# kehlert/ellp

Measured on AMD Instinct MI355X. Metric: simplex pivots/sec (dense LP, primal, tableau resident in HBM), higher is better.
Workload: dtype f64

## Files before the change

### ellp_amd/_engine.py

```python
import ctypes as C
import os

import numpy as np

_HERE = os.path.dirname(os.path.abspath(__file__))
LIB_PATH = os.environ.get("ELLP_HIP_LIB") or os.path.join(_HERE, "libellp_hip.so")

OPTIMAL, INFEASIBLE, UNBOUNDED, MAXITER = 0, 1, 2, 3
ERR_BAD_DIMS, ERR_SINGULAR, ERR_NAN, ERR_DEVICE, ERR_ARG, ERR_PANIC = -1, -2, -3, -4, -5, -6
STATUS_NAME = {0: "optimal", 1: "infeasible", 2: "unbounded", 3: "maxiter", -1: "err_bad_dims",
               -2: "err_singular", -3: "err_nan", -4: "err_device", -5: "err_arg", -6: "err_panic"}
MAX_ITER_NONE = 2**64 - 1
ENGINE_PRIMAL, ENGINE_DUAL = 0, 1
FLAG_DENSE_PRICING, FLAG_DUAL_MAX_VIOLATION, FLAG_PRIMAL_STEEPEST_EDGE, FLAG_NO_CERTIFY, FLAG_DUAL_BOUND_FLIPPING = 1, 2, 4, 8, 16
K_NAMES = ["price", "select", "ftran", "ratio", "update", "btran", "refactor", "dleave", "dprice",
           "dselect", "dupdate", "event_cost"]
K_COUNT = 12
TAP_U, TAP_R, TAP_D, TAP_BINV, TAP_KEY, TAP_ALPHA, TAP_STATE = range(7)
TAP_SE_GAMMA = 7


class Opts(C.Structure):
    _fields_ = [("max_iter", C.c_uint64), ("eps", C.c_double), ("device", C.c_int32),
                ("refactor_period", C.c_int32), ("btran_mode", C.c_int32),
                ("poll_interval", C.c_int32), ("profile", C.c_int32), ("use_graph", C.c_int32),
                ("pipeline", C.c_int32), ("trace_len", C.c_int32), ("partial_segments", C.c_int32),
                ("flags", C.c_int32)]


class Stats(C.Structure):
    _fields_ = [("iters", C.c_uint64), ("pivots", C.c_uint64), ("bound_flips", C.c_uint64),
                ("refactors", C.c_uint64), ("obj", C.c_double), ("t_loop_s", C.c_double),
                ("t_setup_s", C.c_double), ("kernel_ms", C.c_double * K_COUNT),
                ("kernel_calls", C.c_uint64 * K_COUNT)]

    def as_dict(self):
        d = {k: getattr(self, k) for k in ("iters", "pivots", "bound_flips", "refactors", "obj",
                                           "t_loop_s", "t_setup_s")}
        d["kernel_ms"] = {K_NAMES[i]: self.kernel_ms[i] for i in range(K_COUNT) if self.kernel_calls[i]}
        d["kernel_calls"] = {K_NAMES[i]: self.kernel_calls[i] for i in range(K_COUNT) if self.kernel_calls[i]}
        return d


EXCHANGE_FN = C.CFUNCTYPE(C.c_int, C.c_void_p, C.c_void_p, C.c_int64, C.c_int)


class EllpHipError(RuntimeError):
    def __init__(self, status, msg):
        super().__init__(f"{STATUS_NAME.get(status, status)}: {msg}")
        self.status = status
        self.msg = msg


_lib = None
_PROBLEM_ARGS = [C.c_int64, C.c_int64, C.c_int64, C.c_void_p, C.c_void_p, C.c_void_p, C.c_void_p,
                 C.c_void_p, C.c_void_p, C.c_void_p, C.c_void_p, C.c_int64, C.c_void_p, C.c_void_p,
                 C.c_int64]


def lib():
    global _lib
    if _lib is not None:
        return _lib
    if not os.path.exists(LIB_PATH):
        raise ImportError(
            f"{LIB_PATH} is missing: the HIP engine is the only compute path of ellp_amd. "
            "Build it with `python -m ellp_amd.build` (hipcc --offload-arch=gfx950).")
    L = C.CDLL(LIB_PATH, mode=C.RTLD_GLOBAL)
    L.ellp_default_opts.argtypes = [C.POINTER(Opts)]
    L.ellp_hip_device_count.restype = C.c_int
    L.ellp_hip_abi_version.restype = C.c_int
    tail = [C.POINTER(Opts), C.POINTER(Stats), C.c_char_p, C.c_size_t]
    L.ellp_primal_solve_with_initial.restype = C.c_int
    L.ellp_primal_solve_with_initial.argtypes = _PROBLEM_ARGS + tail
    L.ellp_dual_solve_with_initial.restype = C.c_int
    L.ellp_dual_solve_with_initial.argtypes = _PROBLEM_ARGS + [C.c_void_p, C.c_void_p] + tail
    L.ellp_batch_solve_with_initial.restype = C.c_int
    L.ellp_batch_solve_with_initial.argtypes = [C.c_int, C.c_int64, C.c_void_p, C.POINTER(Opts), C.c_void_p, C.c_void_p,
                                                C.c_char_p, C.c_size_t]
    L.ellp_batch_primal_solve.restype = C.c_int
    L.ellp_batch_primal_solve.argtypes = [C.c_int64, C.c_void_p, C.POINTER(Opts), C.c_void_p, C.c_char_p, C.c_size_t]
    L.ellp_batch_primal_info.restype = None
    L.ellp_batch_primal_info.argtypes = [C.c_void_p]
    L.ellp_batch_dual_phase1_start.restype = C.c_int
    L.ellp_batch_dual_phase1_start.argtypes = [C.c_int64, C.c_void_p, C.POINTER(Opts), C.c_void_p, C.c_void_p, C.c_char_p,
                                               C.c_size_t]
    L.ellp_engine_create.restype = C.c_int
    L.ellp_engine_create.argtypes = ([C.c_int] + _PROBLEM_ARGS + [C.c_void_p, C.c_void_p] +
                                     [C.POINTER(Opts), C.POINTER(C.c_void_p), C.c_char_p, C.c_size_t])
    L.ellp_engine_plan.restype = C.c_int
    L.ellp_engine_plan.argtypes = [C.c_int, C.c_int64, C.c_int64, C.POINTER(Opts), C.c_int, C.c_void_p, C.c_int64, C.c_char_p, C.c_size_t]
    L.ellp_engine_run.restype = C.c_int
    L.ellp_engine_run.argtypes = [C.c_void_p, C.c_uint64, C.POINTER(Stats), C.c_char_p, C.c_size_t]
    L.ellp_engine_read_point.restype = C.c_int
    L.ellp_engine_read_point.argtypes = [C.c_void_p] + [C.c_void_p] * 6 + [C.c_char_p, C.c_size_t]
    L.ellp_engine_tap.restype = C.c_int64
    L.ellp_engine_tap.argtypes = [C.c_void_p, C.c_int, C.c_void_p, C.c_int64]
    L.ellp_engine_refactor.restype = C.c_int
    L.ellp_engine_refactor.argtypes = [C.c_void_p, C.c_char_p, C.c_size_t]
    L.ellp_engine_refresh.restype = C.c_double
    L.ellp_engine_refresh.argtypes = [C.c_void_p]
    L.ellp_engine_inverse_residual.restype = C.c_double
# ... 558 lines not shown
```

### ellp_amd/csrc/engine/ellp_engine.hip

```cpp
#include <hip/hip_runtime.h>
#include <dlfcn.h>
#include <rccl/rccl.h>

#include <algorithm>
#include <chrono>
#include <cmath>
#include <cstdarg>
#include <cstdint>
#include <cstdio>
#include <cstdlib>
#include <cstring>
#include <limits>
#include <memory>
#include <mutex>
#include <optional>
#include <vector>

#include "ellp_hip.h"
#include "ellp_lu_dev.h"

namespace {

constexpr int ST_RUNNING = 100;
constexpr int ST_NEED_MAINT = 101;
// ... 1699 lines not shown
    } else {
        const double theta_d = st->s_theta_d, delta = st->s_delta;
        const double theta_p = delta / d_r;
        const double *rho = src + r * a.ld;
        if (blockIdx.x == 0) {
        for (int64_t j0 = tid; j0 < a.nN; j0 += 4 * 256) {
            int64_t v[4];
            double al[4], dv[4];
#pragma unroll
            for (int k = 0; k < 4; ++k) {
                const int64_t j = j0 + 256 * k;
                const bool ok = j < a.nN && j != q;
                v[k] = ok ? a.N_index[j] : -1;
                al[k] = ok ? a.xc.r(j) : 0.0;
            }
#pragma unroll
            for (int k = 0; k < 4; ++k) dv[k] = v[k] >= 0 ? a.dd[v[k]] : 0.0;
#pragma unroll
            for (int k = 0; k < 4; ++k)
                if (v[k] >= 0) a.dd[v[k]] = dv[k] - theta_d * al[k];
        }
        return;
        }
        if (blockIdx.x == 1) {
            const int64_t lv = st->s_lv;
            for (int64_t i = tid; i < m; i += 256) a.y[i] = a.y[i] + theta_d * rho[i];
            swap_columns(a.A_N, a.A_B, q, r, a.ld, tid);
            if (tid == 0) {
                a.dd[lv] = -theta_d;
                a.dd[jq] = 0.0;
                a.N_index[q] = lv;
                a.Nb[q] = (uint8_t)st->s_side;
                const double tc = a.c_N[q];
                a.c_N[q] = a.c_B[r];
                a.c_B[r] = tc;
            }
            return;
        }
        for (int64_t i = tid; i < m; i += 256) {
            const int64_t bi = a.B_index[i];
            a.x[bi] = a.x[bi] - theta_p * a.d[i];
        }
        __syncthreads();
        if (tid == 0) {
            a.x[jq] = a.x[jq] + theta_p;
            st->obj = st->obj + theta_d * delta;
            a.B_index[r] = jq;
            st->cur = cur ^ 1;
            st->pivots += 1;
            st->iters += 1;
            trace_put(a.trace, st->iters, st->obj);
            if (d_r != d_r || theta_p != theta_p) st->status = ELLP_ERR_NAN;
        }
        __syncthreads();
        find_leaving(a.B_index, a.x, a.kind, a.lb, a.ub, a.eps, m, tid, s_tmp, st, a.maxviol);
        if (tid == 0 && tiny_pivot && st->status == ST_RUNNING) st->tiny = 1;
    }
    STAMP(2, 4);
}

struct DLeaveArgs {
    const double *x, *lb, *ub;
    const uint8_t *kind;
    const int64_t *B_index;
    DevState *st;
    int64_t m;
    double eps;
    int maxviol;
};
__global__ __launch_bounds__(256) void k_dleave(DLeaveArgs a) {
    __shared__ long long s_tmp[4];
    if (a.st->status != ST_RUNNING) return;
    find_leaving(a.B_index, a.x, a.kind, a.lb, a.ub, a.eps, a.m, threadIdx.x, s_tmp, a.st, a.maxviol);
}

struct BtranArgs {
    const double *W0, *W1, *c_B;
    double *upart, *u, *u_alt;
    DevState *st;
    int64_t m, ld;
    int rows_per_tile, ntiles;
};

__device__ __forceinline__ void btran_part_body(BtranArgs a, unsigned bx, unsigned by) {
    if (a.st->status != ST_RUNNING) return;
    const int64_t half = a.ld >> 1;
    const int64_t j2 = (int64_t)bx * 256 + threadIdx.x;
    const int64_t i0 = (int64_t)by * a.rows_per_tile;
    const int64_t i1 = (i0 + a.rows_per_tile < a.m) ? i0 + a.rows_per_tile : a.m;
    double2 acc = make_double2(0.0, 0.0);
    if (j2 < half) {
        const double2 *W2 = reinterpret_cast<const double2 *>(a.st->cur ? a.W1 : a.W0);
        for (int64_t i = i0; i < i1; ++i) {
            const double ci = a.c_B[i];
            if (ci != 0.0) {
                const double2 w = W2[i * half + j2];
                acc.x = fma(ci, w.x, acc.x);
                acc.y = fma(ci, w.y, acc.y);
            }
        }
        reinterpret_cast<double2 *>(a.upart)[(int64_t)by * half + j2] = acc;
    }
}
__global__ __launch_bounds__(256) void k_btran_part(BtranArgs a) { btran_part_body(a, blockIdx.x, blockIdx.y); }
__device__ __forceinline__ void btran_reduce_body(BtranArgs a, unsigned bx) {
    if (a.st->status != ST_RUNNING) return;
    const int64_t j = (int64_t)bx * 256 + threadIdx.x;
    if (j >= a.ld) return;
    double s = 0.0;
    int t = 0;
    for (; t + 8 <= a.ntiles; t += 8) {
        double v[8];
#pragma unroll
        for (int k = 0; k < 8; ++k) v[k] = a.upart[(int64_t)(t + k) * a.ld + j];
#pragma unroll
        for (int k = 0; k < 8; ++k) s += v[k];
    }
    for (; t < a.ntiles; ++t) s += a.upart[(int64_t)t * a.ld + j];
    (a.st->usel ? a.u_alt : a.u)[j] = s;
}
__global__ __launch_bounds__(256) void k_btran_reduce(BtranArgs a) { btran_reduce_body(a, blockIdx.x); }


__device__ __forceinline__ double nanmax(double a, double b) { return (a != a) ? a : ((b > a || b != b) ? b : a); }

struct DriftArgs {
    const double *A_B, *A_N, *d;
    const double *aq_cur;
    double *upart;
    DevState *st;
    int64_t m, ld;
    int cols_per_tile, ntiles;
    double tol;
};
__global__ __launch_bounds__(256) void k_drift_part(DriftArgs a) {
    if (a.st->status != ST_RUNNING || a.st->pp_skip) return;
    const int64_t half = a.ld >> 1;
    const int64_t i2 = (int64_t)blockIdx.x * 256 + threadIdx.x;
    const int64_t k0 = (int64_t)blockIdx.y * a.cols_per_tile;
    const int64_t k1 = (k0 + a.cols_per_tile < a.m) ? k0 + a.cols_per_tile : a.m;
    if (i2 >= half) return;
    const double2 *AB2 = reinterpret_cast<const double2 *>(a.A_B);
    double2 acc = make_double2(0.0, 0.0);
    for (int64_t k = k0; k < k1; ++k) {
        const double dk = a.d[k];
        const double2 c = AB2[k * half + i2];
        acc.x = fma(dk, c.x, acc.x);
        acc.y = fma(dk, c.y, acc.y);
    }
    reinterpret_cast<double2 *>(a.upart)[(int64_t)blockIdx.y * half + i2] = acc;
}
__global__ __launch_bounds__(1024) void k_drift_reduce(DriftArgs a) {
    __shared__ double s_r[16], s_s[16];
    DevState *st = a.st;
    if (st->status != ST_RUNNING || st->pp_skip) return;
    const int tid = threadIdx.x, lane = tid & 63, wave = tid >> 6;
    const double sgn = st->s_at_lower ? -1.0 : 1.0;
    const double *aq = a.aq_cur ? a.aq_cur : a.A_N + st->s_q * a.ld;
    double res = 0.0, scale = 0.0;
    for (int64_t i = tid; i < a.m; i += 1024) {
        double t = 0.0;
        for (int k = 0; k < a.ntiles; ++k) t += a.upart[(int64_t)k * a.ld + i];
        const double q = aq[i];
        res = nanmax(res, fabs(sgn * t - q));
        scale = nanmax(scale, fabs(q));
    }
#pragma unroll
    for (int o = 32; o > 0; o >>= 1) {
        res = nanmax(res, __shfl_xor(res, o));
        scale = nanmax(scale, __shfl_xor(scale, o));
    }
    if (lane == 0) {
        s_r[wave] = res;
        s_s[wave] = scale;
    }
    __syncthreads();
    if (tid == 0) {
        for (int w = 1; w < 16; ++w) {
            res = nanmax(res, s_r[w]);
            scale = nanmax(scale, s_s[w]);
        }
        const double rel = res / (scale > 0.0 ? scale : 1.0);
        st->drift = rel;
        if (rel > a.tol || rel != rel) st->tiny = 1;
    }
}

struct ResyncArgs {
    const double *A_N, *W0, *W1, *b;
    double *x, *xg, *tvec, *upart, *cand;
    unsigned long long *maxbits;
    const int64_t *B_index, *N_index;
    DevState *st;
    int64_t m, ld, nN;
    int cols_per_tile, ntiles;
    int force;
};
__device__ __forceinline__ void resync_gather_body(ResyncArgs a, unsigned bx) {
    const int64_t j = (int64_t)bx * 256 + threadIdx.x;
    if (j < a.nN) a.xg[j] = a.x[a.N_index[j]];
}
__global__ __launch_bounds__(256) void k_resync_gather(ResyncArgs a) { resync_gather_body(a, blockIdx.x); }
__device__ __forceinline__ void resync_part_body(ResyncArgs a, unsigned bx, unsigned by) {
    if (a.st->status != ST_RUNNING && a.st->status != ST_NEED_MAINT) return;
    const int64_t half = a.ld >> 1;
    const int64_t i2 = (int64_t)bx * 256 + threadIdx.x;
    const int64_t j0 = (int64_t)by * a.cols_per_tile;
    const int64_t j1 = (j0 + a.cols_per_tile < a.nN) ? j0 + a.cols_per_tile : a.nN;
    if (i2 >= half) return;
    const double2 *AN2 = reinterpret_cast<const double2 *>(a.A_N);
    double2 acc = make_double2(0.0, 0.0);
    for (int64_t j = j0; j < j1; ++j) {
        const double xj = a.xg[j];
        if (xj == 0.0) continue;
        const double2 c = AN2[j * half + i2];
        acc.x = fma(xj, c.x, acc.x);
        acc.y = fma(xj, c.y, acc.y);
    }
    reinterpret_cast<double2 *>(a.upart)[(int64_t)by * half + i2] = acc;
}
__global__ __launch_bounds__(256) void k_resync_part(ResyncArgs a) { resync_part_body(a, blockIdx.x, blockIdx.y); }
__device__ __forceinline__ void resync_rhs_body(ResyncArgs a, unsigned bx) {
    if (a.st->status != ST_RUNNING && a.st->status != ST_NEED_MAINT) return;
    const int64_t i = (int64_t)bx * 256 + threadIdx.x;
    if (i >= a.ld) return;
    double s = 0.0;
    for (int k = 0; k < a.ntiles; ++k) s += a.upart[(int64_t)k * a.ld + i];
    a.tvec[i] = i < a.m ? a.b[i] - s : 0.0;
}
__global__ __launch_bounds__(256) void k_resync_rhs(ResyncArgs a) { resync_rhs_body(a, blockIdx.x); }
__device__ __forceinline__ void resync_xb_body(ResyncArgs a, unsigned bx) {
    if (a.st->status != ST_RUNNING && a.st->status != ST_NEED_MAINT) return;
    const int lane = threadIdx.x & 63;
    const int64_t i = (int64_t)bx * 4 + (threadIdx.x >> 6);
    if (i >= a.m) return;
    const int64_t half = a.ld >> 1;
    const double2 *row = reinterpret_cast<const double2 *>((a.st->cur ? a.W1 : a.W0) + i * a.ld);
    const double2 *t2 = reinterpret_cast<const double2 *>(a.tvec);
    double acc0 = 0.0, acc1 = 0.0;
    for (int64_t t = lane; t < half; t += WAVE) {
        const double2 w = row[t], v = t2[t];
        acc0 = fma(w.x, v.x, acc0);
        acc1 = fma(w.y, v.y, acc1);
    }
    const double r = wave_sum(acc0 + acc1);
    if (lane == 0) {
        const double xo = a.x[a.B_index[i]];
        a.cand[i] = r;
        const double df = fabs(r - xo), ax = fabs(xo);
        if (df == df) atomicMax(&a.maxbits[0], (unsigned long long)__double_as_longlong(df));
        else atomicMax(&a.maxbits[0], 0x7ff0000000000000ull);
        if (ax == ax) atomicMax(&a.maxbits[1], (unsigned long long)__double_as_longlong(ax));
    }
}
__global__ __launch_bounds__(256) void k_resync_xb(ResyncArgs a) { resync_xb_body(a, blockIdx.x); }
__device__ __forceinline__ void resync_apply_body(ResyncArgs a, unsigned bx) {
    if (a.st->status != ST_RUNNING && a.st->status != ST_NEED_MAINT) return;
    if (a.st->need_rebuild) return;
    const double maxdiff = __longlong_as_double((long long)a.maxbits[0]);
    const double maxx = __longlong_as_double((long long)a.maxbits[1]);
    if (!a.force && (!(maxdiff > 1e-11 * (1.0 + maxx)) || isinf(maxdiff))) return;
    const int64_t i = (int64_t)bx * 256 + threadIdx.x;
    if (i < a.m) a.x[a.B_index[i]] = a.cand[i];
}
__global__ __launch_bounds__(256) void k_resync_apply(ResyncArgs a) { resync_apply_body(a, blockIdx.x); }

struct RefArgs {
    double *W0, *W1, *d;
    const double *A_B;
    int32_t *used;
    int64_t *perm;
    DevState *st;
    int64_t m, ld;
    int rows_per_block;
    double eps;
};

__device__ __forceinline__ void ref_init_body(RefArgs a, unsigned bx, unsigned gx) {
    if (a.st->status != ST_RUNNING) return;
    double *W = a.st->cur ? a.W1 : a.W0;
    const int64_t total = a.m * a.ld;
    for (int64_t t = (int64_t)bx * 256 + threadIdx.x; t < total; t += (int64_t)gx * 256) {
        const int64_t i = t / a.ld, j = t - i * a.ld;
        W[t] = (i == j) ? 1.0 : 0.0;
    }
    for (int64_t i = (int64_t)bx * 256 + threadIdx.x; i < a.m; i += (int64_t)gx * 256) a.used[i] = 0;
}
__global__ __launch_bounds__(256) void k_ref_init(RefArgs a) { ref_init_body(a, blockIdx.x, gridDim.x); }
__global__ void k_ref_begin(RefArgs a) {
    if (a.st->status != ST_RUNNING) return;
    a.st->refk = 0;
}

__global__ __launch_bounds__(256) void k_ref_ftran(RefArgs a) {
    if (a.st->status != ST_RUNNING) return;
    const int lane = threadIdx.x & 63;
    const int64_t wave_global = (int64_t)blockIdx.x * 4 + (threadIdx.x >> 6);
    const int64_t nwaves = (int64_t)gridDim.x * 4;
    const int64_t half = a.ld >> 1;
    const double *W = a.st->cur ? a.W1 : a.W0;
    const double2 *col = reinterpret_cast<const double2 *>(a.A_B + a.st->refk * a.ld);
    for (int64_t i = wave_global; i < a.m; i += nwaves) {
        const double2 *row = reinterpret_cast<const double2 *>(W + i * a.ld);
        double acc0 = 0.0, acc1 = 0.0;
        for (int64_t t0 = lane; t0 < half; t0 += 8 * WAVE) {
            double2 w[8], c[8];
#pragma unroll
            for (int u = 0; u < 8; ++u) {
                const int64_t t = t0 + u * WAVE;
                w[u] = t < half ? row[t] : make_double2(0.0, 0.0);
                c[u] = t < half ? col[t] : make_double2(0.0, 0.0);
            }
#pragma unroll
            for (int u = 0; u < 8; ++u) {
                acc0 = fma(w[u].x, c[u].x, acc0);
                acc1 = fma(w[u].y, c[u].y, acc1);
            }
        }
        const double s = wave_sum(acc0 + acc1);
        if (lane == 0) a.d[i] = s;
    }
}

__global__ __launch_bounds__(1024) void k_ref_pick(RefArgs a) {
    __shared__ double s_v[16];
    __shared__ long long s_i[16];
    DevState *st = a.st;
    if (st->status != ST_RUNNING) return;
    const int tid = threadIdx.x, lane = tid & 63, wave = tid >> 6;
    double bv = -1.0;
    long long bi = -1;
    for (int64_t i = tid; i < a.m; i += 1024) {
        if (a.used[i]) continue;
        const double v = fabs(a.d[i]);
        if (v > bv) {
// ... 873 lines not shown
    hipLaunchKernelGGL(k_bl_perm_check, dim3(1), dim3(1024), 0, e->stream, a, e->bl_nzval, e->bl_nzrow, e->bl_nzcnt);
    hipLaunchKernelGGL(k_bl_perm_fill, dim3((unsigned)m), dim3(256), 0, e->stream, a, e->bl_nzval, e->bl_nzrow);
    DevState probe;
    if (hipMemcpyAsync(&probe, e->st, sizeof(DevState), hipMemcpyDeviceToHost, e->stream) != hipSuccess ||
        hipStreamSynchronize(e->stream) != hipSuccess)
        return;
    static const int32_t zero = 0;
    (void)hipMemcpyAsync(&e->st->do_update, &zero, sizeof(int32_t), hipMemcpyHostToDevice, e->stream);
    if (probe.status != ST_RUNNING) return;
    if (probe.do_update) {
        e->rebuild_shortcuts += 1;
        return;
    }
    RefArgs ra{e->W, e->W2, e->d, e->A_B, e->used, e->perm, e->st, e->m, e->ld, e->upd_rows, a.eps};
    hipLaunchKernelGGL(k_ref_init, dim3(1024), dim3(256), 0, e->stream, ra);
    const auto [bl_nt, nbw_max] = bl_factor_variant(m);
    for (int64_t k0 = 0; k0 < m; k0 += BL_NB) {
        a.k0 = (int)k0;
        a.nbc = (int)((m - k0) < BL_NB ? (m - k0) : BL_NB);
        a.sel = 0;
        hipLaunchKernelGGL(k_bl_gemm1, dim3((unsigned)((m + 63) / 64), (unsigned)a.splits), dim3(256), 0, e->stream, a);
        hipLaunchKernelGGL(k_bl_sum, dim3(256), dim3(256), 0, e->stream, a);
        for (int j0 = 0; j0 < a.nbc; j0 += nbw_max) {
            a.j0 = j0;
            a.nbw = (a.nbc - j0) < nbw_max ? (a.nbc - j0) : nbw_max;
            a.nacc = j0;
            if (bl_nt == 512) {
                if (nbw_max == 16) hipLaunchKernelGGL((k_bl_factor<16, 4, 512>), dim3(1), dim3(512), 0, e->stream, a);
                else if (nbw_max == 8) hipLaunchKernelGGL((k_bl_factor<8, 8, 512>), dim3(1), dim3(512), 0, e->stream, a);
                else hipLaunchKernelGGL((k_bl_factor<4, 16, 512>), dim3(1), dim3(512), 0, e->stream, a);
            } else {
                if (nbw_max == 16) hipLaunchKernelGGL((k_bl_factor<16, 2, 1024>), dim3(1), dim3(1024), 0, e->stream, a);
                else if (nbw_max == 8) hipLaunchKernelGGL((k_bl_factor<8, 4, 1024>), dim3(1), dim3(1024), 0, e->stream, a);
                else hipLaunchKernelGGL((k_bl_factor<4, 8, 1024>), dim3(1), dim3(1024), 0, e->stream, a);
            }
            hipLaunchKernelGGL(k_bl_apply, dim3((unsigned)((m + 7) / 8)), dim3(256), 0, e->stream, a);
            a.sel ^= 1;
        }
        hipLaunchKernelGGL(k_bl_gather, dim3((unsigned)a.nbc), dim3(256), 0, e->stream, a);
        hipLaunchKernelGGL(k_bl_gemm2, dim3((unsigned)((e->ld + 127) / 128), (unsigned)((m + 63) / 64)), dim3(256), 0, e->stream, a);
    }
    hipLaunchKernelGGL(k_ref_permute, dim3((unsigned)e->m), dim3(256), 0, e->stream, ra);
    hipLaunchKernelGGL(k_ref_finish, dim3(1), dim3(1), 0, e->stream, ra);
}

void launch_refresh(ellp_engine *e) {
    Prof p(e, ELLP_K_REFACTOR);
    GemmArgs a{e->W, e->W2, e->A_B, e->T, e->resid, e->st, e->m, e->ld};
    const unsigned nt = (unsigned)((e->m + 127) / 128);
    static const bool valu = [] {
        const char *v = getenv("ELLP_GEMM");
        return v && strcmp(v, "valu") == 0;
    }();
    if (valu) hipLaunchKernelGGL(k_gemm128<0>, dim3(nt, nt), dim3(256), 0, e->stream, a);
    else hipLaunchKernelGGL(k_gemm_mfma<0>, dim3(nt, nt), dim3(512), 0, e->stream, a);
    hipLaunchKernelGGL(k_resid_reduce, dim3(1), dim3(256), 0, e->stream, a, (int)(nt * nt));
    if (valu) hipLaunchKernelGGL(k_gemm128<1>, dim3(nt, nt), dim3(256), 0, e->stream, a);
    else hipLaunchKernelGGL(k_gemm_mfma<1>, dim3(nt, nt), dim3(512), 0, e->stream, a);
    hipLaunchKernelGGL(k_copy_to_other, dim3(1024), dim3(256), 0, e->stream, a);
    hipLaunchKernelGGL(k_refresh_finish, dim3(1), dim3(1), 0, e->stream, a);
    e->refreshes += 1;
    e->since_refactor = 0;
    e->u_valid = false;
}

void launch_dleave(ellp_engine *e);
void launch_resync(ellp_engine *e, int force);

ResyncArgs launch_resync_rhs(ellp_engine *e, int force) {
    ResyncArgs a{e->A_N, e->W, e->W2, e->b_dev, e->x, e->xg, e->tvec, e->upart, e->cand, e->maxbits, e->B_index,
                 e->N_index, e->st, e->m, e->ld, e->nN, 0, e->btran_tiles, force};
    a.cols_per_tile = (int)((e->nN + e->btran_tiles - 1) / e->btran_tiles);
    const int64_t half = e->ld >> 1;
    hipLaunchKernelGGL(k_resync_gather, dim3((unsigned)((e->nN + 255) / 256)), dim3(256), 0, e->stream, a);
    hipLaunchKernelGGL(k_resync_part, dim3((unsigned)((half + 255) / 256), (unsigned)e->btran_tiles), dim3(256), 0,
                       e->stream, a);
    hipLaunchKernelGGL(k_resync_rhs, dim3((unsigned)((e->ld + 255) / 256)), dim3(256), 0, e->stream, a);
    return a;
}

void launch_resync(ellp_engine *e, int force) {
    if (e->nN <= 0) return;
    if (e->colshard) return;
    (void)hipMemsetAsync(e->maxbits, 0, 2 * sizeof(unsigned long long), e->stream);
    const ResyncArgs a = launch_resync_rhs(e, force);
    hipLaunchKernelGGL(k_resync_xb, dim3((unsigned)((e->m + 3) / 4)), dim3(256), 0, e->stream, a);
    hipLaunchKernelGGL(k_resync_apply, dim3((unsigned)((e->m + 255) / 256)), dim3(256), 0, e->stream, a);
    if (e->kind == ELLP_ENGINE_DUAL) launch_dleave(e);
    e->resyncs += 1;
    if (getenv("ELLP_RESYNC_DEBUG")) {
        unsigned long long hb[2] = {0, 0};
        (void)hipMemcpyAsync(hb, e->maxbits, sizeof(hb), hipMemcpyDeviceToHost, e->stream);
        (void)hipStreamSynchronize(e->stream);
        double dv[2];
        memcpy(dv, hb, sizeof(dv));
        fprintf(stderr, "ellp resync %llu: max|cand - x_B| %.3e, max|x_B| %.3e\n", (unsigned long long)e->resyncs, dv[0], dv[1]);
    }
}

void launch_dual_close(ellp_engine *e);
void maintain_inverse(ellp_engine *e, bool reactive = false, bool rebuild = false) {
    launch_dual_close(e);
    if (e->lagged) hipLaunchKernelGGL(k_drop_open, dim3(1), dim3(1), 0, e->stream, e->st);
    e->lag_open = false;
    if (rebuild) launch_refactor(e);
    else launch_refresh(e);
    const char *mode = getenv("ELLP_RESYNC");
    const bool want = mode && mode[0] == '0' ? false : (mode && mode[0] == '1' ? reactive : true);
    if (want) launch_resync(e, 0);
}

void reconcile_counters(ellp_engine *e) {
    const uint64_t ran = e->h_st->iters >= e->iters_seen ? e->h_st->iters - e->iters_seen : 0;
    const uint64_t lost = e->enqueued > ran ? e->enqueued - ran : 0;
    if (lost) {
        e->since_refactor = e->since_refactor > lost ? e->since_refactor - lost : 0;
        e->since_btran = e->since_btran > lost ? e->since_btran - lost : 0;
        e->since_drift = e->since_drift > lost ? e->since_drift - lost : 0;
    }
    e->enqueued = 0;
    e->iters_seen = e->h_st->iters;
}

void adopt_fin(ellp_engine *e) {
    if (e->h_st->status != ST_RUNNING || !e->h_st->fin) return;
    static int32_t fin_status;
    fin_status = e->h_st->fin - 1;
    (void)hipMemcpyAsync(&e->st->status, &fin_status, sizeof(int32_t), hipMemcpyHostToDevice, e->stream);
    (void)hipStreamSynchronize(e->stream);
    e->h_st->status = fin_status;
}

bool service_maintenance_request(ellp_engine *e) {
    if (e->h_st->status != ST_NEED_MAINT && !(e->h_st->status == ST_RUNNING && e->h_st->tiny)) return false;
    const int32_t running = ST_RUNNING, zero = 0;
    const bool rebuild = e->h_st->need_rebuild != 0;
    (void)hipMemcpyAsync(&e->st->status, &running, sizeof(int32_t), hipMemcpyHostToDevice, e->stream);
    (void)hipMemcpyAsync(&e->st->tiny, &zero, sizeof(int32_t), hipMemcpyHostToDevice, e->stream);
    (void)hipMemcpyAsync(&e->st->need_rebuild, &zero, sizeof(int32_t), hipMemcpyHostToDevice, e->stream);
    e->h_st->status = ST_RUNNING;
    e->h_st->tiny = 0;
    e->h_st->need_rebuild = 0;
    maintain_inverse(e, true, rebuild);
    e->maint_chain = 1;
    (void)hipStreamSynchronize(e->stream);
    e->maint_requests += 1;
    return true;
}

void launch_drift_check(ellp_engine *e) {
    if (e->drift_every <= 0) return;
    if (++e->since_drift < (uint64_t)e->drift_every) return;
    e->since_drift = 0;
    e->drift_checks += 1;
    DriftArgs a{e->A_B, e->A_N, e->d, e->colshard ? e->aq_cur : nullptr, e->upart, e->st, e->m, e->ld, e->btran_rows, e->btran_tiles, e->drift_tol};
    const int64_t half = e->ld >> 1;
    hipLaunchKernelGGL(k_drift_part, dim3((unsigned)((half + 255) / 256), (unsigned)e->btran_tiles), dim3(256), 0,
                       e->stream, a);
    hipLaunchKernelGGL(k_drift_reduce, dim3(1), dim3(1024), 0, e->stream, a);
}

void launch_price2(ellp_engine *e, int use_pend) {
    Price2Args a{};
    a.p.A_N = e->A_N; a.p.W0 = e->W; a.p.W1 = e->W2; a.p.u = nullptr; a.p.c_N = e->c_N; a.p.Nb = e->Nb;
    a.p.N_index = e->N_index; a.p.dd = nullptr; a.p.xc = Xchg{e->X, e->seg, e->nbs, e->cpb}; a.p.st = e->st;
    a.p.ld = e->ld; a.p.nN = e->nN; a.p.cpb = e->cpb; a.p.block0 = e->rank * e->nbs; a.p.eps = e->eps;
    a.p.vs_row = e->vs_row; a.p.vs_val = e->vs_val; a.pos_hint = e->pos_hint;
    a.u0 = e->u; a.u1 = e->u + e->ld; a.W0 = e->W; a.W1 = e->W2;
    a.d = e->d; a.lam = e->lam; a.bmin = e->bmin; a.bsec = e->bmin + e->m; a.bidx = e->bidx; a.binfo = e->binfo; a.dpos = e->dpos;
    a.A_N = e->A_N; a.A_B = e->A_B; a.aq_save = e->aq_save; a.c_B = e->c_B; a.c_N = e->c_N; a.x = e->x;
    a.lb = e->lb; a.ub = e->ub; a.kind = e->kindv; a.B_index = e->B_index; a.N_index = e->N_index; a.Nb = e->Nb;
    a.m = e->m; a.rpb = e->upd2_rows; a.use_pend = use_pend; a.ill_tol = e->ill_tol;
    a.guard_abs = (e->cert_large && !e->guard_off) ? e->guard_abs : 0.0;
    a.aq_cur = e->colshard ? e->aq_cur : nullptr; a.own0 = e->own0; a.own1 = e->own1;
    a.trace = Trace{e->trace_obj, e->trace_it, e->trace_len};
    int mine = e->nblocks - a.p.block0;
    if (mine > e->nbs) mine = e->nbs;
    if (mine < 0) mine = 0;
    const dim3 g(mine + P2_BOOK), b(256);
    const size_t lds = e->price2_lds;
    if (e->colshard) {
        if (e->price_wave) {
            hipLaunchKernelGGL((k_price2_wave<true>), g, b, lds + sizeof(double) * (size_t)e->ld, e->stream, a);
            return;
        }
        if (e->price_nt) {
            switch (e->priceT) {
            case 1: hipLaunchKernelGGL((k_price2<1, true, true>), g, b, lds, e->stream, a); break;
            case 2: hipLaunchKernelGGL((k_price2<2, true, true>), g, b, lds, e->stream, a); break;
            case 4: hipLaunchKernelGGL((k_price2<4, true, true>), g, b, lds, e->stream, a); break;
            case 8: hipLaunchKernelGGL((k_price2<8, true, true>), g, b, lds, e->stream, a); break;
            default: hipLaunchKernelGGL((k_price2<16, true, true>), g, b, lds, e->stream, a); break;
            }
        } else {
            switch (e->priceT) {
            case 1: hipLaunchKernelGGL((k_price2<1, false, true>), g, b, lds, e->stream, a); break;
            case 2: hipLaunchKernelGGL((k_price2<2, false, true>), g, b, lds, e->stream, a); break;
            case 4: hipLaunchKernelGGL((k_price2<4, false, true>), g, b, lds, e->stream, a); break;
            case 8: hipLaunchKernelGGL((k_price2<8, false, true>), g, b, lds, e->stream, a); break;
            default: hipLaunchKernelGGL((k_price2<16, false, true>), g, b, lds, e->stream, a); break;
            }
        }
        return;
    }
    if (e->price_wave) {
        hipLaunchKernelGGL((k_price2_wave<false>), g, b, lds + sizeof(double) * (size_t)e->ld, e->stream, a);
        return;
    }
    if (e->price_nt) {
        switch (e->priceT) {
        case 1: hipLaunchKernelGGL((k_price2<1, true>), g, b, lds, e->stream, a); break;
        case 2: hipLaunchKernelGGL((k_price2<2, true>), g, b, lds, e->stream, a); break;
        case 4: hipLaunchKernelGGL((k_price2<4, true>), g, b, lds, e->stream, a); break;
        case 8: hipLaunchKernelGGL((k_price2<8, true>), g, b, lds, e->stream, a); break;
        default: hipLaunchKernelGGL((k_price2<16, true>), g, b, lds, e->stream, a); break;
        }
    } else {
        switch (e->priceT) {
        case 1: hipLaunchKernelGGL((k_price2<1, false>), g, b, lds, e->stream, a); break;
        case 2: hipLaunchKernelGGL((k_price2<2, false>), g, b, lds, e->stream, a); break;
        case 4: hipLaunchKernelGGL((k_price2<4, false>), g, b, lds, e->stream, a); break;
        case 8: hipLaunchKernelGGL((k_price2<8, false>), g, b, lds, e->stream, a); break;
        default: hipLaunchKernelGGL((k_price2<16, false>), g, b, lds, e->stream, a); break;
        }
    }
}

void launch_ftran_eta(ellp_engine *e) {
    FtranEtaArgs a{};
    a.W0 = e->W; a.W1 = e->W2; a.A_N = e->A_N; a.xc = Xchg{e->X, e->seg, e->nbs, e->cpb};
    a.N_index = e->N_index; a.B_index = e->B_index; a.Nb = e->Nb; a.kind = e->kindv;
    a.x = e->x; a.lb = e->lb; a.ub = e->ub; a.d = e->d; a.lam = e->lam; a.bmin = e->bmin; a.bsec = e->bmin + e->m; a.bidx = e->bidx;
    a.binfo = e->binfo; a.dpos = e->dpos;
    a.A_B = e->A_B; a.c_B = e->c_B; a.aq_save = e->aq_save; a.st = e->st; a.m = e->m; a.ld = e->ld; a.nN = e->nN;
    a.nblocks = e->nblocks; a.cpb = e->cpb; a.rows_per_block = e->upd2_rows; a.eps = e->eps;
    if (e->colshard) {
        a.aq_cur = e->aq_cur; a.aq_out = e->aq_cur;
        if (e->sel_in_ftran) {
            a.sel_packs = e->packs; a.sel_world = e->world; a.mbox_commit = e->sel_commit ? 1 : 0;
        }
    }
    const dim3 g(e->upd2_blocks + 1), b(256);
// ... 1558 lines not shown
            if (getenv("ELLP_HYBRID_DEBUG"))
                fprintf(stderr, "ellp hybrid: end point violates an invariant (x %.3e, d %.3e, objective %.17g): redo on fresh LUs\n", det[0], det[1], det[2]);
            const ellp_status rs = redo_from_snapshot(e, true, errbuf, errlen);
            if (rs != ELLP_OPTIMAL) return rs;
            result = run_exact_large(e, e->opts.max_iter, errbuf, errlen);
            e->obj_fresh = false;
        } else if (!ok) {
            if (getenv("ELLP_HYBRID_DEBUG"))
                fprintf(stderr, "ellp hybrid: end point violates an invariant (x %.3e, d %.3e, objective %.17g against the carried %.17g): redo\n",
                        det[0], det[1], det[2], e->h_st->obj);
            const ellp_status rs = redo_from_snapshot(e, false, errbuf, errlen);
            if (rs != ELLP_OPTIMAL) return rs;
            result = run_small(e, e->opts.max_iter, errbuf, errlen);
            e->obj_fresh = false;
        }
    }
    if (result == ELLP_MAXITER && e->lag_open && !e->small && e->world == 1 && e->h_st->iters >= e->opts.max_iter) {
        launch_flush(e);
        hipLaunchKernelGGL(k_primal_obj, dim3(1), dim3(1024), 0, e->stream, e->c_B, e->c_N, e->x, e->B_index, e->N_index, e->m,
                           e->nN, e->st);
        HIPCHK(hipMemcpyAsync(e->h_st, e->st, sizeof(DevState), hipMemcpyDeviceToHost, e->stream));
        HIPCHK(hipStreamSynchronize(e->stream));
        reconcile_counters(e);
        adopt_fin(e);
        e->obj_fresh = true;
        if (e->h_st->status != ST_RUNNING && e->h_st->status != ST_NEED_MAINT) result = status_message(*e->h_st, errbuf, errlen);
    }
    if (stats) {
        fill_stats(e, stats);
        stats->t_loop_s = std::chrono::duration<double>(std::chrono::steady_clock::now() - t0).count();
    }
    e->hst_fresh = result == ELLP_MAXITER && !e->small && e->world == 1 && !e->colshard && e->nN > 0 &&
                   e->h_st->status == ST_RUNNING;
    return result;
}

ellp_status ellp_engine_read_point(ellp_engine *e, double *x, int64_t *B_index, int64_t *N_index, uint8_t *N_bound,
                                   double *y, double *d, char *errbuf, size_t errlen) {
    if (e) e->hst_fresh = false;
    if (!e) return ELLP_ERR_ARG;
    HIPCHK(hipSetDevice(e->device));
    const bool was_open = e->lag_open;
    launch_flush(e);
    if (was_open) HIPCHK(hipMemcpyAsync(e->h_st, e->st, sizeof(DevState), hipMemcpyDeviceToHost, e->stream));
    if (x) HIPCHK(hipMemcpyAsync(x, e->x, sizeof(double) * (size_t)e->n_c, hipMemcpyDeviceToHost, e->stream));
    if (B_index) HIPCHK(hipMemcpyAsync(B_index, e->B_index, sizeof(int64_t) * (size_t)e->m, hipMemcpyDeviceToHost, e->stream));
    if (N_index && e->nN) HIPCHK(hipMemcpyAsync(N_index, e->N_index, sizeof(int64_t) * (size_t)e->nN, hipMemcpyDeviceToHost, e->stream));
    if (N_bound && e->nN) HIPCHK(hipMemcpyAsync(N_bound, e->Nb, (size_t)e->nN, hipMemcpyDeviceToHost, e->stream));
    if (e->kind == ELLP_ENGINE_DUAL) {
        if (y) HIPCHK(hipMemcpyAsync(y, e->y, sizeof(double) * (size_t)e->m, hipMemcpyDeviceToHost, e->stream));
        if (d) HIPCHK(hipMemcpyAsync(d, e->dd, sizeof(double) * (size_t)e->n_c, hipMemcpyDeviceToHost, e->stream));
    }
    HIPCHK(hipStreamSynchronize(e->stream));
    if (was_open) {
        adopt_fin(e);
        const int32_t stt = e->h_st->status;
        if (stt != ST_RUNNING && stt != ST_NEED_MAINT && stt != ELLP_OPTIMAL) return status_message(*e->h_st, errbuf, errlen);
    }
    return ELLP_OPTIMAL;
}

int64_t ellp_engine_tap(ellp_engine *e, int what, double *dst, int64_t cap) {
    if (e) e->hst_fresh = false;
    if (!e || !dst) return ELLP_ERR_ARG;
    if (hipSetDevice(e->device) != hipSuccess) return ELLP_ERR_DEVICE;
    if (what != ELLP_TAP_STATE) launch_flush(e);
    const double *src = nullptr;
    int64_t count = 0;
    switch (what) {
    case ELLP_TAP_U:
        if (hipMemcpyAsync(e->h_st, e->st, sizeof(DevState), hipMemcpyDeviceToHost, e->stream) != hipSuccess ||
            hipStreamSynchronize(e->stream) != hipSuccess)
            return ELLP_ERR_DEVICE;
        src = e->u + (e->h_st->usel ? e->ld : 0);
        count = e->m;
        break;
    case ELLP_TAP_R:
    case ELLP_TAP_ALPHA:
        if (e->world != 1) return ELLP_ERR_ARG;
        src = e->X + 2 * e->nbs + (int64_t)e->nbs * e->cpb;
        count = e->nN;
        break;
    case ELLP_TAP_D: src = e->d; count = e->m; break;
    case ELLP_TAP_SE_GAMMA:
        if (!e->se) return ELLP_ERR_ARG;
        src = e->se_gamma;
        count = e->nN;
        break;
    case ELLP_TAP_KEY:
        if (e->world != 1) return ELLP_ERR_ARG;
        src = e->X + 2 * e->nbs;
        count = e->nN;
        break;
    case ELLP_TAP_STATE: {
        if (cap < 12) return ELLP_ERR_ARG;
        if (hipMemcpyAsync(e->h_st, e->st, sizeof(DevState), hipMemcpyDeviceToHost, e->stream) != hipSuccess ||
            hipStreamSynchronize(e->stream) != hipSuccess)
            return ELLP_ERR_DEVICE;
        const DevState &h = *e->h_st;
        const double v[12] = {(double)h.status, (double)h.cur, (double)h.s_q, (double)h.s_r, h.s_theta_d, h.s_delta,
                              (double)h.lr, h.ldelta, (double)h.iters, (double)h.pivots, h.lambda, h.s_rq};
        for (int k = 0; k < 12; ++k) dst[k] = v[k];
        if (cap >= 14) {
            dst[12] = h.drift;
            dst[13] = (double)e->drift_checks;
            if (cap >= 20) {
                dst[14] = (double)e->maint_requests;
                dst[15] = (double)e->refreshes;
                dst[16] = (double)e->refactors;
                dst[17] = (double)e->resyncs;
                dst[18] = h.resid;
                dst[19] = e->small ? 0.0 : ((e->lagged || e->dual_fused) ? 2.0 : 3.0);
                if (cap >= 22) {
                    dst[20] = (double)e->rebuild_shortcuts;
                    dst[21] = e->t_setup;
                    if (cap >= 28) {
                        dst[22] = e->hybrid ? 1.0 : (e->cert_large ? 2.0 : 0.0);
                        dst[23] = (double)e->hy_guards;
                        dst[24] = (double)e->hy_certs;
                        dst[25] = (double)e->hy_disagree;
                        dst[26] = (double)e->hy_exact_iters;
                        dst[27] = (double)e->hy_rebuilds;
                        if (cap >= 29) {
                            dst[28] = (double)e->hy_redos;
                            if (cap >= 30) {
                                dst[29] = (double)e->hy_uncertified;
                                return 30;
                            }
                            return 29;
                        }
                        return 28;
                    }
                    return 22;
                }
                return 20;
            }
            return 14;
        }
        return 12;
    }
    case ELLP_TAP_BINV: {
        count = e->m * e->m;
        if (count > cap) return ELLP_ERR_ARG;
        if (ensure_inverse(e, nullptr, 0) != ELLP_OPTIMAL) return ELLP_ERR_DEVICE;
        if (hipMemcpyAsync(e->h_st, e->st, sizeof(DevState), hipMemcpyDeviceToHost, e->stream) != hipSuccess ||
            hipStreamSynchronize(e->stream) != hipSuccess)
            return ELLP_ERR_DEVICE;
        if (hipMemcpy2DAsync(dst, sizeof(double) * (size_t)e->m, e->h_st->cur ? e->W2 : e->W, sizeof(double) * (size_t)e->ld,
                             sizeof(double) * (size_t)e->m, (size_t)e->m, hipMemcpyDeviceToHost, e->stream) != hipSuccess)
            return ELLP_ERR_DEVICE;
        if (hipStreamSynchronize(e->stream) != hipSuccess) return ELLP_ERR_DEVICE;
        return count;
    }
    default: return ELLP_ERR_ARG;
    }
    if (count > cap) count = cap;
    if (count > 0) {
        if (hipMemcpyAsync(dst, src, sizeof(double) * (size_t)count, hipMemcpyDeviceToHost, e->stream) != hipSuccess)
            return ELLP_ERR_DEVICE;
        if (hipStreamSynchronize(e->stream) != hipSuccess) return ELLP_ERR_DEVICE;
    }
    return count;
}

int64_t ellp_engine_read_trace(ellp_engine *e, uint64_t *iters_out, double *obj_out, int64_t cap) {
    if (e) e->hst_fresh = false;
// ... 1063 lines not shown
```

### include/ellp_hip.h

```cpp
#ifndef ELLP_HIP_H
#define ELLP_HIP_H

#include <stddef.h>
#include <stdint.h>

#ifdef __cplusplus
extern "C" {
#endif

#define ELLP_HIP_ABI_VERSION 1

typedef enum ellp_status {
    ELLP_OPTIMAL = 0,
    ELLP_INFEASIBLE = 1,
    ELLP_UNBOUNDED = 2,
    ELLP_MAXITER = 3,
    ELLP_ERR_BAD_DIMS = -1,
    ELLP_ERR_SINGULAR = -2,
    ELLP_ERR_NAN = -3,
    ELLP_ERR_DEVICE = -4,
    ELLP_ERR_ARG = -5,
    ELLP_ERR_PANIC = -6
} ellp_status;

// ... 112 lines not shown
ellp_status ellp_batch_primal_solve(int64_t count, ellp_batch_primal_item *items, const ellp_opts *opts,
                                    ellp_batch_primal_result *results, char *errbuf, size_t errbuf_len);

void ellp_batch_primal_info(uint64_t *out4);

typedef struct ellp_engine ellp_engine;
enum { ELLP_ENGINE_PRIMAL = 0, ELLP_ENGINE_DUAL = 1 };

ellp_status ellp_engine_create(
    int kind,
    int64_t m, int64_t n, int64_t n_c,
    const double *A, const double *c, const double *b,
    const uint8_t *bound_kind, const double *lb, const double *ub,
    const double *x,
    const int64_t *B_index, int64_t n_B,
    const int64_t *N_index, const uint8_t *N_bound, int64_t n_N,
    const double *y, const double *d,
    const ellp_opts *opts, ellp_engine **out, char *errbuf, size_t errbuf_len);

ellp_status ellp_engine_create_primal_phase1(
    int64_t m, int64_t n,
    const double *A, const double *b,
    const uint8_t *bound_kind, const double *lb, const double *ub,
    const double *x, const uint8_t *N_bound,
    const ellp_opts *opts, ellp_engine **out, char *errbuf, size_t errbuf_len);

ellp_status ellp_engine_run(ellp_engine *e, uint64_t max_iters, ellp_stats *stats,
                            char *errbuf, size_t errbuf_len);

ellp_status ellp_engine_read_point(ellp_engine *e, double *x, int64_t *B_index,
                                   int64_t *N_index, uint8_t *N_bound, double *y, double *d,
                                   char *errbuf, size_t errbuf_len);

int64_t ellp_engine_segment_doubles(ellp_engine *e, int world);
ellp_status ellp_engine_set_shard(ellp_engine *e, int rank, int world, void *exchange_buffer, char *errbuf,
                                  size_t errbuf_len);
ellp_status ellp_engine_exchange_info(ellp_engine *e, void **base, int64_t *seg_doubles, int *rank, int *world);
ellp_status ellp_engine_set_stream(ellp_engine *e, void *hip_stream);
ellp_status ellp_engine_step(ellp_engine *e, int phase, char *errbuf, size_t errbuf_len);
ellp_status ellp_engine_poll(ellp_engine *e, ellp_stats *stats, char *errbuf, size_t errbuf_len);

ellp_status ellp_engine_rephase(ellp_engine *e, const double *c, const uint8_t *bound_kind, const double *lb,
                                const double *ub, char *errbuf, size_t errbuf_len);

ellp_status ellp_engine_create_dual_phase1(int64_t m, int64_t n, const double *A, const double *c, const double *b,
                                           const uint8_t *bound_kind, const double *lb, const double *ub,
                                           const int64_t *B_index, const int64_t *N_index, const ellp_opts *opts,
                                           ellp_engine **out, char *errbuf, size_t errlen);

ellp_status ellp_batch_dual_phase1_start(int64_t count, ellp_batch_item *items, const ellp_opts *opts,
                                         ellp_status *status_out, double *obj_out, char *errbuf, size_t errlen);

ellp_status ellp_engine_dual_rephase(ellp_engine *e, const double *c, const double *b, const uint8_t *bound_kind,
                                     const double *lb, const double *ub, char *errbuf, size_t errbuf_len);

#define ELLP_COMM_ID_BYTES 128
ellp_status ellp_comm_unique_id(const char *rccl_path, void *id_out, char *errbuf, size_t errbuf_len);
ellp_status ellp_engine_comm_init(ellp_engine *e, const char *rccl_path, const void *id, int rank, int world,
                                  char *errbuf, size_t errbuf_len);
ellp_status ellp_engine_run_sharded(ellp_engine *e, uint64_t max_iters, ellp_stats *stats, char *errbuf,
                                    size_t errbuf_len);

typedef int (*ellp_exchange_fn)(void *user, void *host_buffer, int64_t segment_bytes, int world);
ellp_status ellp_engine_shard_columns(ellp_engine *e, int rank, int world, char *errbuf, size_t errbuf_len);
ellp_status ellp_engine_set_exchange_callback(ellp_engine *e, ellp_exchange_fn fn, void *user);
#define ELLP_IPC_HANDLE_BYTES 64
ellp_status ellp_engine_mailbox_export(ellp_engine *e, void *handles_out , char *errbuf, size_t errbuf_len);
ellp_status ellp_engine_mailbox_connect(ellp_engine *e, const void *all_handles , char *errbuf,
                                        size_t errbuf_len);
ellp_status ellp_engine_mailbox_selftest(ellp_engine *e, int rounds, char *errbuf, size_t errbuf_len);
ellp_status ellp_engine_shard_info(ellp_engine *e, double *out6);
int ellp_shard_select_compact(const double *packs, int world, int64_t ld, double eps, int64_t *q, int *src_rank,
                              int *src_slot);
int64_t ellp_shard_pack_doubles(int64_t ld);

int64_t ellp_engine_read_trace(ellp_engine *e, uint64_t *iters_out, double *obj_out, int64_t cap);

#define ELLP_PLAN_FIELDS 47
ellp_status ellp_engine_plan(int kind, int64_t m, int64_t n_N, const ellp_opts *opts, int avail_mask, double *out, int64_t cap,
                             char *errbuf, size_t errbuf_len);

enum { ELLP_TAP_U = 0, ELLP_TAP_R = 1, ELLP_TAP_D = 2, ELLP_TAP_BINV = 3, ELLP_TAP_KEY = 4,
       ELLP_TAP_ALPHA = 5, ELLP_TAP_STATE = 6 ,
       ELLP_TAP_SE_GAMMA = 7  };
int64_t ellp_engine_tap(ellp_engine *e, int what, double *dst, int64_t cap);

double ellp_engine_refresh(ellp_engine *e);

ellp_status ellp_engine_refactor(ellp_engine *e, char *errbuf, size_t errbuf_len);

ellp_status ellp_engine_request_maintenance(ellp_engine *e);

ellp_status ellp_engine_debug_scale_inverse(ellp_engine *e, double factor);

ellp_status ellp_engine_debug_set_inverse(ellp_engine *e, const double *W);

ellp_status ellp_engine_debug_set_x(ellp_engine *e, const double *x);

double ellp_engine_inverse_residual(ellp_engine *e);

void ellp_engine_destroy(ellp_engine *e);

ellp_status ellp_hip_qr_transposed(int64_t m, int64_t nv, const double *A, int64_t *pivot_out, double *rdiag_out,
                                   int device, char *errbuf, size_t errbuf_len);

ellp_status ellp_hip_lu_transposed(int64_t m, int64_t nv, const double *A, int64_t *pivot_out, double *udiag_out,
                                   int device, char *errbuf, size_t errbuf_len);

ellp_status ellp_hip_lu_rows(int64_t m, const double *M_in, int variant, double *factors_out, int64_t *pivot_out,
                             double *udiag_out, int device, char *errbuf, size_t errbuf_len);
double ellp_hip_lu_rows_last_ms(void);

#ifdef __cplusplus
}
#endif
#endif
```

Measured before the change: 26790.

## Batch loads with nonzero compaction in btran/drift/resync tile kernels and parallelize drift reduce

Result: faster. 27290, median of 6 (+1.8%).

```diff
diff --git a/ellp_amd/_engine.py b/ellp_amd/_engine.py
--- a/ellp_amd/_engine.py
+++ b/ellp_amd/_engine.py
@@ -18,6 +18,7 @@
 K_COUNT = 12
 TAP_U, TAP_R, TAP_D, TAP_BINV, TAP_KEY, TAP_ALPHA, TAP_STATE = range(7)
 TAP_SE_GAMMA = 7
+TAP_RESYNC_T, TAP_RESYNC_CAND = 8, 9
 
 
 class Opts(C.Structure):
diff --git a/ellp_amd/csrc/engine/ellp_engine.hip b/ellp_amd/csrc/engine/ellp_engine.hip
--- a/ellp_amd/csrc/engine/ellp_engine.hip
+++ b/ellp_amd/csrc/engine/ellp_engine.hip
@@ -1805,42 +1805,90 @@
     int rows_per_tile, ntiles;
 };
 
+constexpr int TILE_BATCH = 8;
+__device__ __forceinline__ void loaded(double &v) { asm volatile("" : "+v"(v)); }
+__device__ __forceinline__ void loaded(double2 &v) {
+    loaded(v.x);
+    loaded(v.y);
+}
+template <bool SKIP>
+__device__ __forceinline__ double2 tile_stream(const double2 *M2, int64_t half, int64_t c2, bool active, const double *coef,
+                                               int64_t i0, int64_t i1) {
+    __shared__ double s_c[WAVE];
+    __shared__ int s_i[WAVE];
+    __shared__ int s_n;
+    double2 acc = make_double2(0.0, 0.0);
+    for (int64_t base = i0; base < i1; base += WAVE) {
+        if (threadIdx.x < WAVE) {
+            const int lane = threadIdx.x;
+            const int64_t i = base + lane;
+            const double ci = i < i1 ? coef[i] : 0.0;
+            const bool keep = i < i1 && (!SKIP || ci != 0.0);
+            const unsigned long long mask = __ballot(keep);
+            if (keep) {
+                const int p = __popcll(mask & ((1ull << lane) - 1ull));
+                s_c[p] = ci;
+                s_i[p] = lane;
+            }
+            if (lane == 0) s_n = __popcll(mask);
+        }
+        __syncthreads();
+        const int n = s_n;
+        if (active) {
+            const double2 *col = M2 + base * half + c2;
+            for (int k = 0; k < n; k += TILE_BATCH) {
+                double2 w[TILE_BATCH];
+#pragma unroll
+                for (int b = 0; b < TILE_BATCH; ++b) w[b] = col[(int64_t)s_i[k + b < n ? k + b : n - 1] * half];
+#pragma unroll
+                for (int b = 0; b < TILE_BATCH; ++b) loaded(w[b]);
+#pragma unroll
+                for (int b = 0; b < TILE_BATCH; ++b) {
+                    if (k + b < n) {
+                        const double ci = s_c[k + b];
+                        acc.x = fma(ci, w[b].x, acc.x);
+                        acc.y = fma(ci, w[b].y, acc.y);
+                    }
+                }
+            }
+        }
+        __syncthreads();
+    }
+    return acc;
+}
+
+constexpr int FOLD_BATCH = 16;
+__device__ __forceinline__ double fold_tiles(const double *p, int64_t ld, int ntiles) {
+    double s = 0.0;
+    for (int t = 0; t < ntiles; t += FOLD_BATCH) {
+        double v[FOLD_BATCH];
+#pragma unroll
+        for (int b = 0; b < FOLD_BATCH; ++b) v[b] = p[(int64_t)(t + b < ntiles ? t + b : t) * ld];
+#pragma unroll
+        for (int b = 0; b < FOLD_BATCH; ++b) loaded(v[b]);
+#pragma unroll
+        for (int b = 0; b < FOLD_BATCH; ++b)
+            if (t + b < ntiles) s += v[b];
+    }
+    return s;
+}
+
 __device__ __forceinline__ void btran_part_body(BtranArgs a, unsigned bx, unsigned by) {
     if (a.st->status != ST_RUNNING) return;
     const int64_t half = a.ld >> 1;
     const int64_t j2 = (int64_t)bx * 256 + threadIdx.x;
     const int64_t i0 = (int64_t)by * a.rows_per_tile;
     const int64_t i1 = (i0 + a.rows_per_tile < a.m) ? i0 + a.rows_per_tile : a.m;
-    double2 acc = make_double2(0.0, 0.0);
-    if (j2 < half) {
-        const double2 *W2 = reinterpret_cast<const double2 *>(a.st->cur ? a.W1 : a.W0);
-        for (int64_t i = i0; i < i1; ++i) {
-            const double ci = a.c_B[i];
-            if (ci != 0.0) {
-                const double2 w = W2[i * half + j2];
-                acc.x = fma(ci, w.x, acc.x);
-                acc.y = fma(ci, w.y, acc.y);
-            }
-        }
-        reinterpret_cast<double2 *>(a.upart)[(int64_t)by * half + j2] = acc;
-    }
+    const double2 *W2 = reinterpret_cast<const double2 *>(a.st->cur ? a.W1 : a.W0);
+    const double2 acc = tile_stream<true>(W2, half, j2, j2 < half, a.c_B, i0, i1);
+    if (j2 < half) reinterpret_cast<double2 *>(a.upart)[(int64_t)by * half + j2] = acc;
 }
 __global__ __launch_bounds__(256) void k_btran_part(BtranArgs a) { btran_part_body(a, blockIdx.x, blockIdx.y); }
 __device__ __forceinline__ void btran_reduce_body(BtranArgs a, unsigned bx) {
     if (a.st->status != ST_RUNNING) return;
     const int64_t j = (int64_t)bx * 256 + threadIdx.x;
     if (j >= a.ld) return;
-    double s = 0.0;
-    int t = 0;
-    for (; t + 8 <= a.ntiles; t += 8) {
-        double v[8];
-#pragma unroll
-        for (int k = 0; k < 8; ++k) v[k] = a.upart[(int64_t)(t + k) * a.ld + j];
-#pragma unroll
-        for (int k = 0; k < 8; ++k) s += v[k];
-    }
-    for (; t < a.ntiles; ++t) s += a.upart[(int64_t)t * a.ld + j];
-    (a.st->usel ? a.u_alt : a.u)[j] = s;
+    (a.st->usel ? a.u_alt : a.u)[j] = fold_tiles(a.upart + j, a.ld, a.ntiles);
 }
 __global__ __launch_bounds__(256) void k_btran_reduce(BtranArgs a) { btran_reduce_body(a, blockIdx.x); }
 
@@ -1862,31 +1910,28 @@
     const int64_t i2 = (int64_t)blockIdx.x * 256 + threadIdx.x;
     const int64_t k0 = (int64_t)blockIdx.y * a.cols_per_tile;
     const int64_t k1 = (k0 + a.cols_per_tile < a.m) ? k0 + a.cols_per_tile : a.m;
-    if (i2 >= half) return;
-    const double2 *AB2 = reinterpret_cast<const double2 *>(a.A_B);
-    double2 acc = make_double2(0.0, 0.0);
-    for (int64_t k = k0; k < k1; ++k) {
-        const double dk = a.d[k];
-        const double2 c = AB2[k * half + i2];
-        acc.x = fma(dk, c.x, acc.x);
-        acc.y = fma(dk, c.y, acc.y);
-    }
-    reinterpret_cast<double2 *>(a.upart)[(int64_t)blockIdx.y * half + i2] = acc;
-}
-__global__ __launch_bounds__(1024) void k_drift_reduce(DriftArgs a) {
-    __shared__ double s_r[16], s_s[16];
+    if (blockIdx.x == 0 && blockIdx.y == 0 && threadIdx.x == 0) a.st->drift = 0.0;
+    const double2 acc = tile_stream<false>(reinterpret_cast<const double2 *>(a.A_B), half, i2, i2 < half, a.d, k0, k1);
+    if (i2 < half) reinterpret_cast<double2 *>(a.upart)[(int64_t)blockIdx.y * half + i2] = acc;
+}
+__global__ __launch_bounds__(WAVE) void k_drift_reduce(DriftArgs a) {
     DevState *st = a.st;
     if (st->status != ST_RUNNING || st->pp_skip) return;
-    const int tid = threadIdx.x, lane = tid & 63, wave = tid >> 6;
+    const int lane = threadIdx.x;
+    const int64_t i = (int64_t)blockIdx.x * WAVE + lane;
     const double sgn = st->s_at_lower ? -1.0 : 1.0;
     const double *aq = a.aq_cur ? a.aq_cur : a.A_N + st->s_q * a.ld;
     double res = 0.0, scale = 0.0;
-    for (int64_t i = tid; i < a.m; i += 1024) {
-        double t = 0.0;
-        for (int k = 0; k < a.ntiles; ++k) t += a.upart[(int64_t)k * a.ld + i];
-        const double q = aq[i];
-        res = nanmax(res, fabs(sgn * t - q));
-        scale = nanmax(scale, fabs(q));
+    for (int64_t r0 = lane; r0 < a.m; r0 += 8 * WAVE) {
+        double q[8];
+#pragma unroll
+        for (int b = 0; b < 8; ++b) q[b] = aq[r0 + b * WAVE < a.m ? r0 + b * WAVE : r0];
+#pragma unroll
+        for (int b = 0; b < 8; ++b) scale = nanmax(scale, fabs(q[b]));
+    }
+    if (i < a.m) {
+        const double t = fold_tiles(a.upart + i, a.ld, a.ntiles);
+        res = nanmax(res, fabs(sgn * t - aq[i]));
     }
 #pragma unroll
     for (int o = 32; o > 0; o >>= 1) {
@@ -1894,17 +1939,8 @@
         scale = nanmax(scale, __shfl_xor(scale, o));
     }
     if (lane == 0) {
-        s_r[wave] = res;
-        s_s[wave] = scale;
-    }
-    __syncthreads();
-    if (tid == 0) {
-        for (int w = 1; w < 16; ++w) {
-            res = nanmax(res, s_r[w]);
-            scale = nanmax(scale, s_s[w]);
-        }
         const double rel = res / (scale > 0.0 ? scale : 1.0);
-        st->drift = rel;
+        atomicMax(reinterpret_cast<unsigned long long *>(&st->drift), (unsigned long long)__double_as_longlong(rel));
         if (rel > a.tol || rel != rel) st->tiny = 1;
     }
 }
@@ -1930,25 +1966,16 @@
     const int64_t i2 = (int64_t)bx * 256 + threadIdx.x;
     const int64_t j0 = (int64_t)by * a.cols_per_tile;
     const int64_t j1 = (j0 + a.cols_per_tile < a.nN) ? j0 + a.cols_per_tile : a.nN;
-    if (i2 >= half) return;
-    const double2 *AN2 = reinterpret_cast<const double2 *>(a.A_N);
-    double2 acc = make_double2(0.0, 0.0);
-    for (int64_t j = j0; j < j1; ++j) {
-        const double xj = a.xg[j];
-        if (xj == 0.0) continue;
-        const double2 c = AN2[j * half + i2];
-        acc.x = fma(xj, c.x, acc.x);
-        acc.y = fma(xj, c.y, acc.y);
-    }
-    reinterpret_cast<double2 *>(a.upart)[(int64_t)by * half + i2] = acc;
+    const double2 acc = tile_stream<true>(reinterpret_cast<const double2 *>(a.A_N), half, i2, i2 < half, a.xg, j0, j1);
+    if (i2 < half) reinterpret_cast<double2 *>(a.upart)[(int64_t)by * half + i2] = acc;
 }
 __global__ __launch_bounds__(256) void k_resync_part(ResyncArgs a) { resync_part_body(a, blockIdx.x, blockIdx.y); }
 __device__ __forceinline__ void resync_rhs_body(ResyncArgs a, unsigned bx) {
+    if (bx == 0 && threadIdx.x == 0) a.maxbits[0] = a.maxbits[1] = 0ull;
     if (a.st->status != ST_RUNNING && a.st->status != ST_NEED_MAINT) return;
     const int64_t i = (int64_t)bx * 256 + threadIdx.x;
     if (i >= a.ld) return;
-    double s = 0.0;
-    for (int k = 0; k < a.ntiles; ++k) s += a.upart[(int64_t)k * a.ld + i];
+    const double s = fold_tiles(a.upart + i, a.ld, a.ntiles);
     a.tvec[i] = i < a.m ? a.b[i] - s : 0.0;
 }
 __global__ __launch_bounds__(256) void k_resync_rhs(ResyncArgs a) { resync_rhs_body(a, blockIdx.x); }
@@ -1961,19 +1988,39 @@
     const double2 *row = reinterpret_cast<const double2 *>((a.st->cur ? a.W1 : a.W0) + i * a.ld);
     const double2 *t2 = reinterpret_cast<const double2 *>(a.tvec);
     double acc0 = 0.0, acc1 = 0.0;
-    for (int64_t t = lane; t < half; t += WAVE) {
-        const double2 w = row[t], v = t2[t];
-        acc0 = fma(w.x, v.x, acc0);
-        acc1 = fma(w.y, v.y, acc1);
+    for (int64_t t0 = lane; t0 < half; t0 += 8 * WAVE) {
+        double2 w[8], v[8];
+#pragma unroll
+        for (int b = 0; b < 8; ++b) {
+            const int64_t t = t0 + b * WAVE < half ? t0 + b * WAVE : t0;
+            w[b] = row[t];
+            v[b] = t2[t];
+        }
+#pragma unroll
+        for (int b = 0; b < 8; ++b) {
+            loaded(w[b]);
+            loaded(v[b]);
+        }
+#pragma unroll
+        for (int b = 0; b < 8; ++b) {
+            if (t0 + b * WAVE < half) {
+                acc0 = fma(w[b].x, v[b].x, acc0);
+                acc1 = fma(w[b].y, v[b].y, acc1);
+            }
+        }
     }
     const double r = wave_sum(acc0 + acc1);
     if (lane == 0) {
         const double xo = a.x[a.B_index[i]];
         a.cand[i] = r;
         const double df = fabs(r - xo), ax = fabs(xo);
-        if (df == df) atomicMax(&a.maxbits[0], (unsigned long long)__double_as_longlong(df));
-        else atomicMax(&a.maxbits[0], 0x7ff0000000000000ull);
-        if (ax == ax) atomicMax(&a.maxbits[1], (unsigned long long)__double_as_longlong(ax));
+        const unsigned long long dbits = df == df ? (unsigned long long)__double_as_longlong(df)
+                                                  : 0x7ff0000000000000ull;
+        if (dbits > __atomic_load_n(&a.maxbits[0], __ATOMIC_RELAXED)) atomicMax(&a.maxbits[0], dbits);
+        if (ax == ax) {
+            const unsigned long long xbits = (unsigned long long)__double_as_longlong(ax);
+            if (xbits > __atomic_load_n(&a.maxbits[1], __ATOMIC_RELAXED)) atomicMax(&a.maxbits[1], xbits);
+        }
     }
 }
 __global__ __launch_bounds__(256) void k_resync_xb(ResyncArgs a) { resync_xb_body(a, blockIdx.x); }
@@ -3013,7 +3060,6 @@
 void launch_resync(ellp_engine *e, int force) {
     if (e->nN <= 0) return;
     if (e->colshard) return;
-    (void)hipMemsetAsync(e->maxbits, 0, 2 * sizeof(unsigned long long), e->stream);
     const ResyncArgs a = launch_resync_rhs(e, force);
     hipLaunchKernelGGL(k_resync_xb, dim3((unsigned)((e->m + 3) / 4)), dim3(256), 0, e->stream, a);
     hipLaunchKernelGGL(k_resync_apply, dim3((unsigned)((e->m + 255) / 256)), dim3(256), 0, e->stream, a);
@@ -3088,7 +3134,7 @@
     const int64_t half = e->ld >> 1;
     hipLaunchKernelGGL(k_drift_part, dim3((unsigned)((half + 255) / 256), (unsigned)e->btran_tiles), dim3(256), 0,
                        e->stream, a);
-    hipLaunchKernelGGL(k_drift_reduce, dim3(1), dim3(1024), 0, e->stream, a);
+    hipLaunchKernelGGL(k_drift_reduce, dim3((unsigned)((e->m + WAVE - 1) / WAVE)), dim3(WAVE), 0, e->stream, a);
 }
 
 void launch_price2(ellp_engine *e, int use_pend) {
@@ -4813,6 +4859,8 @@
         count = e->nN;
         break;
     case ELLP_TAP_D: src = e->d; count = e->m; break;
+    case ELLP_TAP_RESYNC_T: src = e->tvec; count = e->m; break;
+    case ELLP_TAP_RESYNC_CAND: src = e->cand; count = e->m; break;
     case ELLP_TAP_SE_GAMMA:
         if (!e->se) return ELLP_ERR_ARG;
         src = e->se_gamma;
diff --git a/include/ellp_hip.h b/include/ellp_hip.h
--- a/include/ellp_hip.h
+++ b/include/ellp_hip.h
@@ -218,7 +218,9 @@
 
 enum { ELLP_TAP_U = 0, ELLP_TAP_R = 1, ELLP_TAP_D = 2, ELLP_TAP_BINV = 3, ELLP_TAP_KEY = 4,
        ELLP_TAP_ALPHA = 5, ELLP_TAP_STATE = 6 ,
-       ELLP_TAP_SE_GAMMA = 7  };
+       ELLP_TAP_SE_GAMMA = 7 ,
+       ELLP_TAP_RESYNC_T = 8 ,
+       ELLP_TAP_RESYNC_CAND = 9  };
 int64_t ellp_engine_tap(ellp_engine *e, int what, double *dst, int64_t cap);
 
 double ellp_engine_refresh(ellp_engine *e);
```
